# David-Wobrock/image-processing-graph-laplacian

Measured on AMD Instinct MI355X. Metric: filtered Mpixels/sec @ 4K img, 0.5% samples; PSNR vs PETSc ref, higher is better.
Workload: dtype f32 (f32 storage and accumulation; MFMA operands split into f16 hi+lo pairs = 22 significant bits)

## Files before the change

image-processing-graph-laplacian_amd/csrc/ctx.hip:

```cpp
#include "glf_internal.hpp"

#include <cmath>
#include <cstdlib>

extern "C" {

const char *glf_strerror(int status)
{
    switch (status) {
    case GLF_OK: return "ok";
    case GLF_ERR_INVALID: return "invalid argument";
    case GLF_ERR_NOMEM: return "out of memory";
    case GLF_ERR_HIP: return "HIP runtime error";
    case GLF_ERR_NODEVICE: return "no usable gfx950 device";
    case GLF_ERR_COMM: return "collective callback failed";
    case GLF_ERR_NOCONV: return "eigensolver did not converge";
    case GLF_ERR_IO: return "image I/O error";
    case GLF_ERR_UNSUPPORTED: return "unsupported";
    default: return "unknown status";
    }
}

int glf_ctx_create(glf_ctx **out, int device, void *hip_stream)
{
// ... 125 lines not shown
{
    if (!ctx) return GLF_OK;
    (void)hipSetDevice(ctx->device);
    (void)hipStreamSynchronize(ctx->stream);
    for (auto &e : ctx->ev)
        if (e) (void)hipEventDestroy(e);
    for (auto &row : ctx->mv_ev)
        for (auto &e : row)
            if (e) (void)hipEventDestroy(e);
    for (auto &row : ctx->cp_ev)
        for (auto &e : row)
            if (e) (void)hipEventDestroy(e);
    glf::native_comm_release(ctx);
    if (ctx->mv_scratch) (void)hipFree(ctx->mv_scratch);
    if (ctx->x0_block) (void)hipFree(ctx->x0_block);
    glf::band_cache_free(ctx);
    if (ctx->rank_ftab) (void)hipFree(ctx->rank_ftab);
    if (ctx->rank_ff) (void)hipFree(ctx->rank_ff);
    if (ctx->pinned) (void)hipHostFree(ctx->pinned);
    glf::pool_free_all(ctx, false);
    if (ctx->owns_stream && ctx->stream) (void)hipStreamDestroy(ctx->stream);
    delete ctx;
    return GLF_OK;
}

int glf_ctx_synchronize(glf_ctx *ctx)
{
    if (!ctx) return GLF_ERR_INVALID;
    GLF_HIP(ctx, hipStreamSynchronize(ctx->stream));
    return GLF_OK;
// ... 306 lines not shown
```

image-processing-graph-laplacian_amd/csrc/eigen.hip:

```cpp
#include "glf_internal.hpp"

#include <algorithm>
#include <cmath>
#include <cstdlib>
#include <cstring>

namespace glf {

typedef float f32x16 __attribute__((ext_vector_type(16)));


template <int MB>
__global__ __launch_bounds__(256) void k_block_matvec(const float *__restrict__ A, int64_t lda, unsigned p,
                                                       unsigned p32, const float *__restrict__ X,
                                                       float *__restrict__ Y)
{
    constexpr int LD = MB * 32;
    __shared__ __attribute__((aligned(16))) float xs[2][32 * LD];
    const int lane = threadIdx.x & 63, wave = threadIdx.x >> 6;
    const int half = lane >> 5, l31 = lane & 31;
    const unsigned row = blockIdx.x * 128 + wave * 32 + l31;
    const unsigned rowc = row < p ? row : p - 1;
    const float *arow = A + (size_t)rowc * lda + 16 * half;

// ... 336 lines not shown
    GLF_LAUNCH_CHECK(ctx);
    return GLF_OK;
}

int start_block_cached(glf_ctx *ctx, unsigned p, unsigned m, unsigned ld, unsigned long long seed, const float **d_block)
{
    if (!ctx->x0_block || ctx->x0_p != p || ctx->x0_m != m || ctx->x0_ld != ld || ctx->x0_seed != seed) {
        const size_t n = (size_t)round_up(p, VEC_PAD) * ld;
        std::vector<double> x0((size_t)m * p);
        glf_random_vectors(x0.data(), p, m, seed);
        std::vector<float> h(n, 0.f);
        for (unsigned j = 0; j < m; ++j)
            for (unsigned i = 0; i < p; ++i) h[(size_t)i * ld + j] = (float)x0[(size_t)j * p + i];
        if (ctx->x0_block) (void)hipFree(ctx->x0_block);
        ctx->x0_block = nullptr;
        GLF_HIP(ctx, hipMalloc(reinterpret_cast<void **>(&ctx->x0_block), n * sizeof(float)));
        GLF_HIP(ctx, hipMemcpyAsync(ctx->x0_block, h.data(), n * sizeof(float), hipMemcpyHostToDevice, ctx->stream));
        GLF_HIP(ctx, hipStreamSynchronize(ctx->stream));
        ctx->x0_p = p;
        ctx->x0_m = m;
        ctx->x0_ld = ld;
        ctx->x0_seed = seed;
    }
    *d_block = ctx->x0_block;
    return GLF_OK;
}

int mv_collect(glf_ctx *ctx)
{
    if (ctx->mv_pending == 0) return GLF_OK;
// ... 12 lines not shown
    unsigned r0 = 0, r1 = 0;
    bool dist = false;
    unsigned n() const { return r1 - r0; }
};
static inline Rows rows_of(unsigned p, const MatShard *sh)
{
    Rows r;
    if (sh && sh->rows_per_rank) {
        r.r0 = sh->row0;
        r.r1 = sh->row1;
        r.dist = true;
    } else {
        r.r1 = p;
    }
    return r;
}
static int allreduce_d(glf_ctx *ctx, double *d, size_t n)
{
    if (!ctx->has_comm || ctx->comm.allreduce_sum_f64(ctx->comm.user, d, n) != 0)
        return set_error(ctx, GLF_ERR_COMM, "allreduce_sum_f64 callback failed");
    return GLF_OK;
}
static int allreduce_f(glf_ctx *ctx, float *d, size_t n)
{
    if (!ctx->has_comm || ctx->comm.allreduce_sum_f32(ctx->comm.user, d, n) != 0)
        return set_error(ctx, GLF_ERR_COMM, "allreduce_sum_f32 callback failed");
    return GLF_OK;
}
static int allgather_rows(glf_ctx *ctx, float *V, const MatShard *sh, unsigned ld)
{
// ... 337 lines not shown
    {
        shard = sh;
        rows = rows_of(p, sh);
        const size_t n = (size_t)vec_rows(p, sh, ctx->comm.size) * ld;
        GLF_TRY(R.alloc(ctx, n));
        GLF_TRY(P.alloc(ctx, n));
        GLF_TRY(AP.alloc(ctx, n));
        GLF_TRY(Xs.alloc(ctx, n));
        GLF_TRY(dinv.alloc(ctx, p));
        nblk = (int)ceil_div(rows.n(), RED_ROWS);
        GLF_TRY(partial.alloc(ctx, (size_t)std::max(1, nblk) * 2 * ld));
        GLF_TRY(pmax.alloc(ctx, (size_t)std::max(1, nblk) * ld));
        GLF_TRY(sums.alloc(ctx, (size_t)2 * ld));
        GLF_TRY(scal.alloc(ctx, (size_t)4 * ld));
        GLF_TRY(flags.alloc(ctx, ld + 1));
        for (float *q : {R.p, P.p, AP.p, Xs.p}) GLF_HIP(ctx, hipMemsetAsync(q, 0, n * sizeof(float), ctx->stream));
        s.rz = scal.p;
        s.bn2 = scal.p + ld;
        s.alpha = scal.p + 2 * ld;
        s.beta = scal.p + 3 * ld;
        s.active = flags.p;
        if (!ctx_pinned(ctx)) return set_error(ctx, GLF_ERR_NOMEM, "pinned host page");
        h_nactive = reinterpret_cast<int *>(ctx_pinned(ctx) + PINNED_NACTIVE);
        s.nactive = h_nactive;
        return GLF_OK;
    }
};

static int block_pcg_work(glf_ctx *ctx, CgWork &w, const float *A, int64_t lda, unsigned p, float *XB, unsigned m,
                          unsigned ld, double rtol, int max_it, int *iters, bool solution_to_XB = true)
{
    const int nblk = w.nblk;
    const Rows rows = w.rows;
    const unsigned nloc = rows.n();
    const size_t off = (size_t)rows.r0 * ld;
    hipStream_t st = ctx->stream;
    const dim3 red2(red2_grid(ld)), red2_threads(RED2_THREADS);
    const bool carry = w.carry_maxima && !rows.dist;
    const ColMaxima pmax{w.pmax.p, nblk};
    auto reduce2 = [&](int nv, const double **src, int *src_blk) -> int {
        *src = w.partial.p;
        *src_blk = nblk;
        if (!rows.dist) return GLF_OK;
        if (nv == 1) hipLaunchKernelGGL(k_sum_partials_nv<1>, red2, red2_threads, 0, st, w.partial.p, nblk, ld, w.sums.p);
        else hipLaunchKernelGGL(k_sum_partials_nv<2>, red2, red2_threads, 0, st, w.partial.p, nblk, ld, w.sums.p);
// ... 1 lines not shown
        GLF_TRY(allreduce_d(ctx, w.sums.p, (size_t)nv * ld));
        *src = w.sums.p;
        *src_blk = 1;
        return GLF_OK;
    };
    const double *src = nullptr;
    int src_blk = 0;
    if (nblk > 0)
        hipLaunchKernelGGL(k_cg_init, dim3(nblk), dim3(256), 0, st, XB + off, w.dinv.p + rows.r0, w.R.p + off, w.P.p + off, w.Xs.p + off,
                           nloc, ld, w.partial.p, w.pmax.p);
    GLF_TRY(reduce2(2, &src, &src_blk));
    hipLaunchKernelGGL(k_cg_init_scalars, red2, red2_threads, 0, st, src, src_blk, ld, m, w.s);
    hipLaunchKernelGGL(k_cg_count, dim3(1), dim3(256), 0, st, w.s, ld);
    GLF_LAUNCH_CHECK(ctx);
    int it = 0;
    GLF_HIP(ctx, hipStreamSynchronize(st));
    while (*(volatile int *)w.h_nactive > 0 && it < max_it) {
        ++it;
        if (rows.dist) GLF_TRY(allgather_rows(ctx, w.P.p, w.shard, ld));
        unsigned wn = ld;
        if (w.shard && w.shard->grid && ld >= 64 && !ctx->tune.no_narrow) {
            const int na = *w.h_nactive;
            const unsigned cand = na <= 32 ? 32u : (unsigned)round_up(na, 64);
            if (cand < ld) wn = cand;
        }
        if (wn < ld) {
            if (!w.Pc.p) {
                const size_t n = (size_t)vec_rows(p, w.shard, ctx->comm.size) * ld;
                GLF_TRY(w.Pc.alloc(ctx, n));
                GLF_TRY(w.APc.alloc(ctx, n));
                GLF_TRY(w.pcmax.alloc(ctx, (size_t)ceil_div(p, RED_ROWS) * ld));
                GLF_HIP(ctx, hipMemsetAsync(w.Pc.p, 0, n * sizeof(float), st));
            }
            const ColMaxima pcmax{w.pcmax.p, (int)ceil_div(p, RED_ROWS)};
            hipLaunchKernelGGL(k_cg_pack, dim3((unsigned)pcmax.nblk), dim3(256), 0, st, w.P.p, w.s.active, p, ld, wn, w.Pc.p, w.pcmax.p);
            GLF_TRY(block_matvec(ctx, A, lda, p, w.Pc.p, w.APc.p, wn, w.shard, carry ? &pcmax : nullptr));
            if (nblk > 0)
// ... 3 lines not shown
        } else {
            GLF_TRY(block_matvec(ctx, A, lda, p, w.P.p, w.AP.p, ld, w.shard, carry ? &pmax : nullptr));
        }
        if (nblk > 0) hipLaunchKernelGGL(k_cg_dot, dim3(nblk), dim3(256), 0, st, w.P.p + off, w.AP.p + off, nloc, ld, w.partial.p);
        GLF_TRY(reduce2(1, &src, &src_blk));
        hipLaunchKernelGGL(k_cg_alpha, red2, red2_threads, 0, st, src, src_blk, ld, w.s);
        if (nblk > 0)
            hipLaunchKernelGGL(k_cg_update, dim3(nblk), dim3(256), 0, st, w.Xs.p + off, w.R.p + off, w.P.p + off, w.AP.p + off,
                               w.dinv.p + rows.r0, nloc, ld, w.s, w.partial.p);
        GLF_TRY(reduce2(2, &src, &src_blk));
        hipLaunchKernelGGL(k_cg_beta, red2, red2_threads, 0, st, src, src_blk, ld, rtol * rtol, w.s);
        hipLaunchKernelGGL(k_cg_pupdate, dim3((unsigned)std::max(1, nblk)), dim3(256), 0, st, w.P.p + off, w.R.p + off, w.dinv.p + rows.r0, nloc, ld,
                           w.s, carry ? w.pmax.p : nullptr);
        GLF_LAUNCH_CHECK(ctx);
        GLF_HIP(ctx, hipStreamSynchronize(st));
        if (ctx->tune.verbose) fprintf(stderr, "[glf] block PCG step %d: %d of %u columns active\n", it, *w.h_nactive, m);
    }
    if (nloc > 0 && solution_to_XB)
        GLF_HIP(ctx, hipMemcpyAsync(XB + off, w.Xs.p + off, sizeof(float) * (size_t)nloc * ld, hipMemcpyDeviceToDevice, st));
    if (iters) *iters = it;
    return (*w.h_nactive > 0) ? set_error(ctx, GLF_ERR_NOCONV, "block PCG: %d columns unconverged after %d iterations",
                                          *w.h_nactive, it)
                              : GLF_OK;
}

static int cg_setup(glf_ctx *ctx, CgWork &cg, const float *A, int64_t lda, unsigned p, unsigned ld, const MatShard *shard, const float *d_dinv)
{
    GLF_TRY(cg.init(ctx, p, ld, shard));
    cg.carry_maxima = true;
    if (d_dinv)
// ... 191 lines not shown
            b[u] = rowb[cb + u];
        }
#pragma unroll
        for (int u = 0; u < E; ++u)
#pragma unroll
            for (int v = 0; v < E; ++v) acc[u][v] = fma((double)a[u], (double)b[v], acc[u][v]);
    }
    double *out = Gpart + (size_t)blockIdx.x * ld * ld;
#pragma unroll
    for (int u = 0; u < E; ++u)
#pragma unroll
        for (int v = 0; v < E; ++v) out[(size_t)(ca + u) * ld + cb + v] = acc[u][v];
}

typedef double f64x4 __attribute__((ext_vector_type(4)));
template <int TILE>
__global__ __launch_bounds__(64) void k_gsf_gram_mfma(const float *__restrict__ X, unsigned n, unsigned ld,
                                                       double *__restrict__ Gpart, const float *__restrict__ Y = nullptr)
{
    constexpr int S = TILE / 16;
    const int mb = ld / TILE;
    const int ta = blockIdx.y / mb, tb = blockIdx.y % mb;
    if (!Y && tb < ta) return;
    const float *Yp = Y ? Y : X;
    const int lane = threadIdx.x, l15 = lane & 15, lq = lane >> 4;
    f64x4 acc[S][S];
#pragma unroll
    for (int u = 0; u < S; ++u)
#pragma unroll
        for (int v = 0; v < S; ++v)
#pragma unroll
            for (int r = 0; r < 4; ++r) acc[u][v][r] = 0.0;
    const unsigned r0 = blockIdx.x * GSF_ROWS, r1 = min(r0 + GSF_ROWS, n);
    const float *xa = X + ta * TILE + l15, *yb = Yp + tb * TILE + l15;
    const bool sym = !Y && ta == tb;
    for (unsigned ib = r0; ib < r1; ib += 32) {
        float a[8][S], b[8][S];
#pragma unroll
        for (int q = 0; q < 8; ++q) {
            const unsigned i = min(ib + 4 * q + lq, r1 - 1);
#pragma unroll
            for (int u = 0; u < S; ++u) {
                a[q][u] = xa[(size_t)i * ld + 16 * u];
                b[q][u] = yb[(size_t)i * ld + 16 * u];
            }
        }
#pragma unroll
        for (int q = 0; q < 8; ++q) {
            const bool ok = ib + 4 * q + lq < r1;
            double da[S], db[S];
#pragma unroll
            for (int u = 0; u < S; ++u) {
                da[u] = ok ? (double)a[q][u] : 0.0;
                db[u] = ok ? (double)b[q][u] : 0.0;
            }
#pragma unroll
            for (int u = 0; u < S; ++u)
#pragma unroll
                for (int v = 0; v < S; ++v)
                    if (!sym || v >= u) acc[u][v] = __builtin_amdgcn_mfma_f64_16x16x4f64(da[u], db[v], acc[u][v], 0, 0, 0);
        }
    }
    double *out = Gpart + (size_t)blockIdx.x * ld * ld;
#pragma unroll
    for (int u = 0; u < S; ++u)
#pragma unroll
        for (int v = 0; v < S; ++v) {
            if (sym && v < u) continue;
#pragma unroll
            for (int r = 0; r < 4; ++r) {
                const size_t ga = (size_t)(ta * TILE + 16 * u + lq + 4 * r), gb = (size_t)(tb * TILE + 16 * v + l15);
                out[ga * ld + gb] = acc[u][v][r];
                if (sym && v > u) out[gb * ld + ga] = acc[u][v][r];
            }
        }
}

__global__ __launch_bounds__(256) void k_gsf_sum(const double *__restrict__ Gpart, int nchunks, unsigned ld, int tile,
                                                  double *__restrict__ G, int full = 0)
{
    __shared__ double sh[256];
    const unsigned e = blockIdx.x * 64 + (threadIdx.x & 63);
    const int part = threadIdx.x >> 6;
    const unsigned a = e / ld, b = e % ld;
    const bool live = e < ld * ld && (full || b / tile >= a / tile);
    double s = 0.0;
    if (live) {
        int c = part;
        for (; c + 28 < nchunks; c += 32) {
            double x[8];
// ... 173 lines not shown
            const double tv = ts[j * ld + col];
#pragma unroll
            for (int q = 0; q < 8; ++q) acc[q] = fma((double)xs[(rl + q * nrl) * ld + j0 + j], tv, acc[q]);
        }
    }
    (void)rpt;
    if (col < m)
#pragma unroll
        for (int q = 0; q < 8; ++q) {
            const unsigned i = r0 + rl + q * nrl;
            if (i < n) Out[(size_t)i * ld + col] = (float)acc[q];
        }
}

template <int LD>
__global__ __launch_bounds__(256) void k_gsf_apply_mfma(const float *X, const float *__restrict__ S, float *Out, unsigned n, unsigned m,
                                                         const double *__restrict__ Tn, const int *__restrict__ flag, int tiles)
{
    if (*flag) return;
    constexpr int NTL = LD / 16, TS = LD + 4;
    __shared__ double ts[LD * TS];
    for (unsigned e = threadIdx.x; e < LD * LD; e += 256) ts[(e / LD) * TS + e % LD] = Tn[e];
    __syncthreads();
    const int lane = threadIdx.x & 63, wave = threadIdx.x >> 6, l15 = lane & 15, lq = lane >> 4;
#pragma unroll 1
    for (int tile = 0; tile < tiles; ++tile) {
        const unsigned row0 = (blockIdx.x * 4 * tiles + wave * tiles + tile) * 16;
        if (row0 >= n) break;
        const unsigned ra = min(row0 + l15, n - 1);
        float4 xa[NTL];
#pragma unroll
        for (int jb = 0; jb < NTL; ++jb) xa[jb] = *reinterpret_cast<const float4 *>(X + (size_t)ra * LD + 16 * jb + 4 * lq);
        if (S)
#pragma unroll
            for (int jb = 0; jb < NTL; ++jb) {
                const float4 s4 = *reinterpret_cast<const float4 *>(S + (size_t)ra * LD + 16 * jb + 4 * lq);
                xa[jb] = make_float4(xa[jb].x - s4.x, xa[jb].y - s4.y, xa[jb].z - s4.z, xa[jb].w - s4.w);
            }
        f64x4 acc[NTL];
#pragma unroll
        for (int t = 0; t < NTL; ++t)
#pragma unroll
            for (int r = 0; r < 4; ++r) acc[t][r] = 0.0;
#pragma unroll
        for (int jb = 0; jb < NTL; ++jb) {
            const double a4[4] = {(double)xa[jb].x, (double)xa[jb].y, (double)xa[jb].z, (double)xa[jb].w};
#pragma unroll
            for (int sk = 0; sk < 4; ++sk)
#pragma unroll
                for (int t = jb; t < NTL; ++t)
                    acc[t] = __builtin_amdgcn_mfma_f64_16x16x4f64(a4[sk], ts[(16 * jb + 4 * lq + sk) * TS + 16 * t + l15], acc[t], 0, 0, 0);
        }
#pragma unroll
        for (int t = 0; t < NTL; ++t)
#pragma unroll
            for (int r = 0; r < 4; ++r) {
                const unsigned i = row0 + lq + 4 * r;
                if (i < n && 16 * t + l15 < (int)m) Out[(size_t)i * LD + 16 * t + l15] = (float)acc[t][r];
            }
    }
}

__global__ __launch_bounds__(256) void k_gsf_sub(float *__restrict__ Y, const float *__restrict__ X, unsigned n, unsigned ld, unsigned ma,
                                                  const double *__restrict__ Cm)
{
    __shared__ float xs[GSF_APPLY_TILE];
    __shared__ double ts[4096];
    const unsigned rows = GSF_APPLY_TILE / ld, jb = min(4096u / ld, ld);
    const unsigned r0 = blockIdx.x * rows;
    const unsigned col = threadIdx.x % ld, rl = threadIdx.x / ld, nrl = 256 / ld;
    for (unsigned e = threadIdx.x; e < rows * ld; e += 256) {
        const unsigned i = r0 + e / ld;
        xs[e] = i < n ? X[(size_t)i * ld + e % ld] : 0.f;
    }
// ... 7 lines not shown
        const unsigned jn = min(jb, ma - j0);
        for (unsigned j = 0; j < jn; ++j) {
            const double tv = ts[j * ld + col];
#pragma unroll
            for (int q = 0; q < 8; ++q) acc[q] = fma((double)xs[(rl + q * nrl) * ld + j0 + j], tv, acc[q]);
        }
    }
#pragma unroll
    for (int q = 0; q < 8; ++q) {
        const unsigned i = r0 + rl + q * nrl;
        if (i < n) Y[(size_t)i * ld + col] = (float)((double)Y[(size_t)i * ld + col] - acc[q]);
    }
}

static void launch_gsf_apply(hipStream_t st, const float *X, const float *S, float *out, unsigned n, unsigned ld, unsigned m, const double *Tn,
                             const int *flag)
{
    const int tiles = (int)std::max<int64_t>(1, std::min<int64_t>(4, ceil_div(n, 16 * 4 * 256)));
    const unsigned rows_wg = 16 * 4 * (unsigned)tiles;
    if (ld == 64)
        hipLaunchKernelGGL(k_gsf_apply_mfma<64>, dim3((unsigned)ceil_div(n, rows_wg)), dim3(256), 0, st, X, S, out, n, m, Tn, flag, tiles);
    else if (ld == 32)
        hipLaunchKernelGGL(k_gsf_apply_mfma<32>, dim3((unsigned)ceil_div(n, rows_wg)), dim3(256), 0, st, X, S, out, n, m, Tn, flag, tiles);
    else
        hipLaunchKernelGGL(k_gsf_apply, dim3((unsigned)ceil_div(n, GSF_APPLY_TILE / ld)), dim3(256), 0, st, X, S, out, n, ld, m, Tn, flag);
}

struct GsFusedWork {
    DevBuf<double> Gpart, G, S, Tn;
    DevBuf<int> flag;
    int *h_flag = nullptr;
    int nchunks = 0;
    unsigned n = 0, ld = 0;
    int init(glf_ctx *ctx, unsigned n_, unsigned ld_)
    {
        if (n == n_ && ld == ld_) return GLF_OK;
        n = n_;
        ld = ld_;
        nchunks = (int)ceil_div(n, GSF_ROWS);
        GLF_TRY(Gpart.alloc(ctx, (size_t)std::max(1, nchunks) * ld * ld));
// ... 33 lines not shown
    const float *R;
    float *AX;
};

static int orthonormalise_fused_dev(glf_ctx *ctx, GsFusedWork &f, float *X, Rows rows, unsigned m, unsigned ld,
                                    double *d_norms, int *fell_back, const GsDerive *der = nullptr)
{
    hipStream_t st = ctx->stream;
    const unsigned n = rows.n();
    float *Xout = X + (size_t)rows.r0 * ld;
    const float *Xl = der ? der->Y + (size_t)rows.r0 * ld : Xout;
    GLF_TRY(f.init(ctx, n, ld));
    const int tile = ld >= 64 ? 64 : 32, mb = (int)ld / tile;
    if (f.nchunks > 0) {
        if (tile == 64)
            hipLaunchKernelGGL((k_gsf_gram_mfma<64>), dim3(f.nchunks, mb * mb), dim3(64), 0, st, Xl, n, ld, f.Gpart.p);
        else
            hipLaunchKernelGGL((k_gsf_gram_mfma<32>), dim3(f.nchunks, mb * mb), dim3(64), 0, st, Xl, n, ld, f.Gpart.p);
    }
    hipLaunchKernelGGL(k_gsf_sum, dim3((ld * ld + 63) / 64), dim3(256), 0, st, f.Gpart.p, f.nchunks, ld, tile, f.G.p);
    GLF_LAUNCH_CHECK(ctx);
    if (rows.dist) GLF_TRY(allreduce_d(ctx, f.G.p, (size_t)ld * ld));
    if (ld <= 64)
        hipLaunchKernelGGL(k_gsf_recur_lds, dim3(1), dim3(256), 0, st, ld, m, f.G.p, f.Tn.p, d_norms, f.flag.p, f.h_flag);
    else
        hipLaunchKernelGGL(k_gsf_recur_global, dim3(1), dim3(256), 0, st, ld, m, f.G.p, f.S.p, f.Tn.p, d_norms, f.flag.p, f.h_flag);
    if (n > 0 && der)
        launch_gsf_apply(st, Xout, der->R + (size_t)rows.r0 * ld, der->AX + (size_t)rows.r0 * ld, n, ld, m, f.Tn.p, f.flag.p);
    if (n > 0)
        launch_gsf_apply(st, Xl, nullptr, Xout, n, ld, m, f.Tn.p, f.flag.p);
    GLF_LAUNCH_CHECK(ctx);
    GLF_HIP(ctx, hipStreamSynchronize(st));
    *fell_back = *(volatile int *)f.h_flag;
    return GLF_OK;
}

static int orthonormalise_seq_dev(glf_ctx *ctx, GsWork &w, float *X, unsigned n, unsigned m, unsigned ld)
{
    hipStream_t st = ctx->stream;
    for (unsigned k = 0; k < m; ++k) {
        if (k > 0) {
            hipLaunchKernelGGL(k_gs_dots, dim3(w.nblk), dim3(256), 0, st, X, n, ld, k, w.partial.p);
            hipLaunchKernelGGL(k_gs_fin, dim3(k), dim3(256), 0, st, w.partial.p, w.normpart.p, w.nblk, ld, k, m, w.q.p, w.coef.p);
        }
        hipLaunchKernelGGL(k_gs_apply, dim3(w.nblk), dim3(256), 0, st, X, n, ld, k, w.nblk, w.coef.p, w.normpart.p);
    }
    hipLaunchKernelGGL(k_gs_fin, dim3(m), dim3(256), 0, st, w.partial.p, w.normpart.p, w.nblk, ld, m, m, w.q.p, w.coef.p);
    hipLaunchKernelGGL(k_gs_norms, dim3(1), dim3(256), 0, st, w.q.p, m, w.norms.p);
    hipLaunchKernelGGL(k_scale_all, dim3((unsigned)ceil_div((int64_t)n * ld, 256)), dim3(256), 0, st, X, n, ld, m, w.norms.p);
    GLF_LAUNCH_CHECK(ctx);
// ... 211 lines not shown

struct ResWork {
    DevBuf<float> AX, Gpart, G;
    DevBuf<double> partial, sums;
    double *h_sums = nullptr;
    int nchunks = 0;
    Rows rows;
    const MatShard *shard = nullptr;
    int init(glf_ctx *ctx, unsigned p, unsigned ld, const MatShard *sh = nullptr)
    {
        shard = sh;
        rows = rows_of(p, sh);
        const size_t vr = vec_rows(p, sh, ctx->comm.size);
        nchunks = (int)ceil_div(rows.n(), GRAM_ROWS);
        GLF_TRY(AX.alloc(ctx, vr * ld));
        GLF_HIP(ctx, hipMemsetAsync(AX.p, 0, sizeof(float) * vr * ld, ctx->stream));
        GLF_TRY(Gpart.alloc(ctx, (size_t)std::max(1, nchunks) * ld * ld));
        GLF_TRY(G.alloc(ctx, (size_t)ld * ld));
        GLF_TRY(partial.alloc(ctx, (size_t)std::max<int64_t>(1, ceil_div(rows.n(), RED_ROWS)) * ld));
        GLF_TRY(sums.alloc(ctx, ld));
        if (!ctx_pinned(ctx) || ld > 256) return set_error(ctx, GLF_ERR_NOMEM, "pinned host page");
        h_sums = reinterpret_cast<double *>(ctx_pinned(ctx) + PINNED_SUMS);
        return GLF_OK;
    }
};

static int residual_dev(glf_ctx *ctx, ResWork &w, const float *A, int64_t lda, unsigned p, float *X, unsigned m,
                        unsigned ld, double *h_out, bool ax_ready = false)
{
    const Rows rows = w.rows;
    const unsigned nloc = rows.n();
// ... 42 lines not shown
                            const double *h_X0, int opti_gs, double epsilon, double inner_rtol, int max_outer,
                            float *d_eigvecs, double *h_eigvals, glf_eig_stats *stats, const MatShard *shard,
                            const float *d_dinv, const float *d_X0_block)
{
    if (m == 0 || m > p || !valid_ld(ld) || m > ld)
        return set_error(ctx, GLF_ERR_INVALID, "inverse_power_iteration: m=%u ld=%u p=%u (m <= 256 supported)", m, ld, p);
    if (opti_gs < 1) opti_gs = 1;
    const unsigned p32 = (unsigned)round_up(p, VEC_PAD);
    const size_t n = (size_t)vec_rows(p, shard, ctx->comm.size) * ld;
    const size_t n_out = (size_t)p32 * ld;
    hipStream_t st = ctx->stream;

    DevBuf<float> X, Xb;
    GLF_TRY(X.alloc(ctx, n));
    GLF_TRY(Xb.alloc(ctx, n));
    if (d_X0_block) {
        GLF_HIP(ctx, hipMemsetAsync(X.p, 0, sizeof(float) * n, st));
        GLF_HIP(ctx, hipMemcpyAsync(X.p, d_X0_block, sizeof(float) * n_out, hipMemcpyDeviceToDevice, st));
    } else {
        std::vector<double> own;
        if (!h_X0) {
            own.resize((size_t)m * p);
            glf_random_vectors(own.data(), p, m, 1);
            h_X0 = own.data();
        }
        std::vector<float> h(n, 0.f);
        for (unsigned j = 0; j < m; ++j)
            for (unsigned i = 0; i < p; ++i) h[(size_t)i * ld + j] = (float)h_X0[(size_t)j * p + i];
        GLF_HIP(ctx, hipMemcpyAsync(X.p, h.data(), sizeof(float) * n, hipMemcpyHostToDevice, st));
        GLF_HIP(ctx, hipStreamSynchronize(st));
    }
    GsWork gs;
    GLF_TRY(gs.init(ctx, p, ld));
    CgWork cg;
    GLF_TRY(cg_setup(ctx, cg, A, lda, p, ld, shard, d_dinv));
    ResWork rs;
    GLF_TRY(rs.init(ctx, p, ld, shard));
    const Rows rows = rows_of(p, shard);
    const unsigned nloc = rows.n();
    const size_t off = (size_t)rows.r0 * ld, nloc_ld = (size_t)nloc * ld;
    GLF_TRY(mv_collect(ctx));
    const int mv_count0 = ctx->mv_count, narrow0 = ctx->narrow_sweeps;
    const double mv_ms0 = ctx->mv_ms, mv_bytes0 = ctx->mv_bytes;
    bool replicated = false;
    GLF_TRY(orthonormalise_dev(ctx, gs, X.p, p, m, ld, rows, shard, &replicated));
    GLF_HIP(ctx, hipMemcpyAsync(Xb.p, X.p, sizeof(float) * n, hipMemcpyDeviceToDevice, st));
    double r_norm = 0.0;
    GLF_TRY(residual_dev(ctx, rs, A, lda, p, X.p, m, ld, &r_norm));
    const bool verbose = ctx->tune.verbose;
    if (verbose) fprintf(stderr, "[glf rank %d] initial residual %.9g\n", ctx->comm.rank, r_norm);
    int it = 0, inner_total = 0, rc = GLF_OK;
    const bool derive_ax = !ctx->tune.residual_sweep;
    const bool swap_blocks = derive_ax && !ctx->tune.gs_seq && opti_gs == 1 && !rows.dist;
    while (r_norm > epsilon) {
        if (it >= max_outer) {
            rc = set_error(ctx, GLF_ERR_NOCONV, "inverse iteration: residual %g > %g after %d outer iterations", r_norm,
                           epsilon, it);
            break;
        }
        ++it;
        int inner = 0;
        bool ax_ready = derive_ax;
        if (swap_blocks) {
            GLF_TRY(block_pcg_work(ctx, cg, A, lda, p, X.p, m, ld, inner_rtol, 10 * (int)p + 100, &inner, false));
            inner_total += inner;
            const GsDerive der{cg.Xs.p, cg.R.p, rs.AX.p};
            int fell_back = 0;
            GLF_TRY(orthonormalise_fused_dev(ctx, gs.fused, X.p, rows, m, ld, gs.norms.p, &fell_back, &der));
            gs.last_fused = !fell_back;
            if (fell_back) {
                if (verbose) fprintf(stderr, "[glf] Gram-Schmidt: ill-conditioned block, column-by-column sweep\n");
                GLF_HIP(ctx, hipMemcpyAsync(X.p, cg.Xs.p, sizeof(float) * nloc_ld, hipMemcpyDeviceToDevice, st));
                GLF_TRY(orthonormalise_seq_dev(ctx, gs, X.p, p, m, ld));
                ax_ready = false;
            }
            std::swap(cg.Xs.p, Xb.p);
        } else {
            if (derive_ax && nloc) GLF_HIP(ctx, hipMemcpyAsync(rs.AX.p + off, X.p + off, sizeof(float) * nloc_ld, hipMemcpyDeviceToDevice, st));
            GLF_TRY(block_pcg_work(ctx, cg, A, lda, p, X.p, m, ld, inner_rtol, 10 * (int)p + 100, &inner));
            inner_total += inner;
            if (nloc) GLF_HIP(ctx, hipMemcpyAsync(Xb.p + off, X.p + off, sizeof(float) * nloc_ld, hipMemcpyDeviceToDevice, st));
            if (derive_ax && nloc)
                hipLaunchKernelGGL(k_sub_inplace, dim3((unsigned)ceil_div((int64_t)nloc_ld, 256)), dim3(256), 0, st, rs.AX.p + off, cg.R.p + off, nloc_ld);
            if (it % opti_gs == 0) {
                GLF_TRY(orthonormalise_dev(ctx, gs, X.p, p, m, ld, rows, shard, &replicated));
                if (ax_ready && gs.last_fused) {
                    if (nloc) launch_gsf_apply(st, rs.AX.p + off, nullptr, rs.AX.p + off, nloc, ld, m, gs.fused.Tn.p, gs.fused.flag.p);
                } else {
                    ax_ready = false;
                }
            }
        }
        GLF_LAUNCH_CHECK(ctx);
        GLF_TRY(residual_dev(ctx, rs, A, lda, p, X.p, m, ld, &r_norm, ax_ready));
        if (verbose)
            fprintf(stderr, "[glf rank %d] outer iteration %d: %d block-CG steps, residual %.9g\n", ctx->comm.rank, it, inner, r_norm);
    }
    if (opti_gs != 1 && (it % opti_gs) != 0)
        GLF_TRY(orthonormalise_dev(ctx, gs, X.p, p, m, ld, rows, shard, &replicated));

    if (h_eigvals) {
        std::vector<double> nr(m);
        GLF_HIP(ctx, hipMemcpyAsync(nr.data(), gs.norms.p, sizeof(double) * m, hipMemcpyDeviceToHost, st));
        GLF_HIP(ctx, hipStreamSynchronize(st));
        for (unsigned j = 0; j < m; ++j) h_eigvals[j] = 1.0 / nr[j];
    }
    if (d_eigvecs) {
        GLF_TRY(normalise_dev(ctx, Xb.p, p, m, ld, gs.partial.p, gs.norms.p, rows, cg.sums.p));
        if (rows.dist) GLF_TRY(allgather_rows(ctx, Xb.p, shard, ld));
        GLF_HIP(ctx, hipMemcpyAsync(d_eigvecs, Xb.p, sizeof(float) * n_out, hipMemcpyDeviceToDevice, st));
    }
    GLF_HIP(ctx, hipStreamSynchronize(st));
// ... 215 lines not shown
```

image-processing-graph-laplacian_amd/csrc/glf_internal.hpp:

```cpp
#pragma once

#include <hip/hip_runtime.h>

#include <cmath>
#include <cstdarg>
#include <cstdint>
#include <cstdio>
#include <cstring>
#include <limits>
#include <type_traits>
#include <utility>
#include <vector>

#include "../../include/glf.h"
#include "band_plan.hpp"

struct glf_pool_block {
    void *p;
    size_t bytes;
    bool in_use;
    unsigned last_call = 0;
};

struct glf_tuning {
// ... 35 lines not shown
    hipEvent_t ev[8] = {};
    void *mv_scratch = nullptr;
    size_t mv_scratch_bytes = 0;
    static constexpr int MV_RING = 64;
    hipEvent_t mv_ev[2][MV_RING] = {};
    static constexpr int CP_RING = 16;
    hipEvent_t cp_ev[2][CP_RING] = {};
    int mv_pending = 0;
    unsigned call_no = 0;
    int mv_count = 0;
    int narrow_sweeps = 0;
    double mv_ms = 0.0, mv_bytes = 0.0;
    float *x0_block = nullptr;
    unsigned x0_p = 0, x0_m = 0, x0_ld = 0;
    unsigned long long x0_seed = 0;
    int contraction = GLF_CONTRACT_F16_SPLIT;
    struct { int skipping = 0, lut = 0; } nys_note;
    struct { int path = 0, shape = 0, skipping = 0, chunks = 0, mgroups = 0; double entries = 0.0; } deg_note;
    struct { unsigned kernels = 0, ld = 0, panels = 0, proj_blocks = 0, apply_blocks = 0, strided = 0; } flt_note;
    void *pinned = nullptr;
    void *band_cache[2] = {nullptr, nullptr};
    bool rank_valid = false;
    float rank_s_val = 0.f;
    int rank_R = 0;
    void *rank_ftab = nullptr;
    void *rank_ff = nullptr;
    bool pool_debug = false;
    int pool_violations = 0;
    glf_tuning tune;
};
// ... 662 lines not shown
```

Measured before the change: 2648.

## Cut eigensolver syncs, cache orthonormal start block, widen Gram kernel, fuse apply passes

Several eigensolver changes land together. The orthonormalised random start block and its norms are cached across calls, since they depend only on the seed and shape. The first block-PCG step skips its host sync, the fused Gram-Schmidt no longer waits on its fallback flag before the residual is launched, and buffer memsets now clear only the padding rows. The Gram kernel spreads its MFMA tile pairs over four waves, and the apply kernel writes both orthonormalised outputs in one launch. Together these aim to remove host round trips and redundant passes, at the cost of more control-flow complexity and an extra persistent cache that must be invalidated correctly.

```diff
diff --git a/image-processing-graph-laplacian_amd/csrc/ctx.hip b/image-processing-graph-laplacian_amd/csrc/ctx.hip
--- a/image-processing-graph-laplacian_amd/csrc/ctx.hip
+++ b/image-processing-graph-laplacian_amd/csrc/ctx.hip
@@ -163,6 +163,8 @@
     glf::native_comm_release(ctx);
     if (ctx->mv_scratch) (void)hipFree(ctx->mv_scratch);
     if (ctx->x0_block) (void)hipFree(ctx->x0_block);
+    if (ctx->x0_orth) (void)hipFree(ctx->x0_orth);
+    if (ctx->x0_orth_norms) (void)hipFree(ctx->x0_orth_norms);
     glf::band_cache_free(ctx);
     if (ctx->rank_ftab) (void)hipFree(ctx->rank_ftab);
     if (ctx->rank_ff) (void)hipFree(ctx->rank_ff);
diff --git a/image-processing-graph-laplacian_amd/csrc/eigen.hip b/image-processing-graph-laplacian_amd/csrc/eigen.hip
--- a/image-processing-graph-laplacian_amd/csrc/eigen.hip
+++ b/image-processing-graph-laplacian_amd/csrc/eigen.hip
@@ -374,6 +374,7 @@
             for (unsigned i = 0; i < p; ++i) h[(size_t)i * ld + j] = (float)x0[(size_t)j * p + i];
         if (ctx->x0_block) (void)hipFree(ctx->x0_block);
         ctx->x0_block = nullptr;
+        ctx->x0_orth_form = 0;
         GLF_HIP(ctx, hipMalloc(reinterpret_cast<void **>(&ctx->x0_block), n * sizeof(float)));
         GLF_HIP(ctx, hipMemcpyAsync(ctx->x0_block, h.data(), n * sizeof(float), hipMemcpyHostToDevice, ctx->stream));
         GLF_HIP(ctx, hipStreamSynchronize(ctx->stream));
@@ -416,6 +417,11 @@
         r.r1 = p;
     }
     return r;
+}
+static int zero_pad_rows(glf_ctx *ctx, float *q, size_t from, size_t rows, unsigned ld)
+{
+    if (from < rows) GLF_HIP(ctx, hipMemsetAsync(q + from * ld, 0, (rows - from) * ld * sizeof(float), ctx->stream));
+    return GLF_OK;
 }
 static int allreduce_d(glf_ctx *ctx, double *d, size_t n)
 {
@@ -783,7 +789,8 @@
         GLF_TRY(sums.alloc(ctx, (size_t)2 * ld));
         GLF_TRY(scal.alloc(ctx, (size_t)4 * ld));
         GLF_TRY(flags.alloc(ctx, ld + 1));
-        for (float *q : {R.p, P.p, AP.p, Xs.p}) GLF_HIP(ctx, hipMemsetAsync(q, 0, n * sizeof(float), ctx->stream));
+        const bool may_narrow = sh && sh->grid && ld >= 64 && !ctx->tune.no_narrow;
+        for (float *q : {R.p, P.p, AP.p, Xs.p}) GLF_TRY(zero_pad_rows(ctx, q, (rows.dist || (q == AP.p && may_narrow)) ? 0 : p, n / ld, ld));
         s.rz = scal.p;
         s.bn2 = scal.p + ld;
         s.alpha = scal.p + 2 * ld;
@@ -797,7 +804,7 @@
 };
 
 static int block_pcg_work(glf_ctx *ctx, CgWork &w, const float *A, int64_t lda, unsigned p, float *XB, unsigned m,
-                          unsigned ld, double rtol, int max_it, int *iters, bool solution_to_XB = true)
+                          unsigned ld, double rtol, int max_it, int *iters, bool solution_to_XB = true, bool rhs_active = false)
 {
     const int nblk = w.nblk;
     const Rows rows = w.rows;
@@ -829,13 +836,14 @@
     hipLaunchKernelGGL(k_cg_count, dim3(1), dim3(256), 0, st, w.s, ld);
     GLF_LAUNCH_CHECK(ctx);
     int it = 0;
-    GLF_HIP(ctx, hipStreamSynchronize(st));
-    while (*(volatile int *)w.h_nactive > 0 && it < max_it) {
+    bool unsynced = rhs_active && !rows.dist && !ctx->tune.verbose && max_it > 0;
+    if (!unsynced) GLF_HIP(ctx, hipStreamSynchronize(st));
+    while ((unsynced || *(volatile int *)w.h_nactive > 0) && it < max_it) {
         ++it;
         if (rows.dist) GLF_TRY(allgather_rows(ctx, w.P.p, w.shard, ld));
         unsigned wn = ld;
         if (w.shard && w.shard->grid && ld >= 64 && !ctx->tune.no_narrow) {
-            const int na = *w.h_nactive;
+            const int na = unsynced ? (int)m : *w.h_nactive;
             const unsigned cand = na <= 32 ? 32u : (unsigned)round_up(na, 64);
             if (cand < ld) wn = cand;
         }
@@ -869,6 +877,7 @@
                            w.s, carry ? w.pmax.p : nullptr);
         GLF_LAUNCH_CHECK(ctx);
         GLF_HIP(ctx, hipStreamSynchronize(st));
+        unsynced = false;
         if (ctx->tune.verbose) fprintf(stderr, "[glf] block PCG step %d: %d of %u columns active\n", it, *w.h_nactive, m);
     }
     if (nloc > 0 && solution_to_XB)
@@ -1090,66 +1099,91 @@
 }
 
 typedef double f64x4 __attribute__((ext_vector_type(4)));
+constexpr int GSF_GRAM_WAVES = 4;
+template <int S, bool SYM>
+__host__ __device__ constexpr int gsf_pair_index(int u, int v)
+{
+    return SYM ? u * S - u * (u - 1) / 2 + (v - u) : u * S + v;
+}
+template <int TILE, bool SYM, int W>
+__device__ __forceinline__ void gsf_gram_wave(const float *__restrict__ xa, const float *__restrict__ yb, unsigned ld, unsigned r0,
+                                              unsigned r1, int lq, int l15, int ca, int cb, double *__restrict__ out)
+{
+    constexpr int S = TILE / 16;
+    auto mine = [](int u, int v) { return (!SYM || v >= u) && gsf_pair_index<S, SYM>(u, v) % GSF_GRAM_WAVES == W; };
+    f64x4 acc[S][S];
+#pragma unroll
+    for (int u = 0; u < S; ++u)
+#pragma unroll
+        for (int v = 0; v < S; ++v)
+#pragma unroll
+            for (int r = 0; r < 4; ++r) acc[u][v][r] = 0.0;
+    for (unsigned ib = r0; ib < r1; ib += 32) {
+        float a[8][S], b[8][S];
+#pragma unroll
+        for (int q = 0; q < 8; ++q) {
+            const unsigned i = min(ib + 4 * q + lq, r1 - 1);
+#pragma unroll
+            for (int u = 0; u < S; ++u) {
+                a[q][u] = xa[(size_t)i * ld + 16 * u];
+                b[q][u] = SYM ? a[q][u] : yb[(size_t)i * ld + 16 * u];
+            }
+        }
+#pragma unroll
+        for (int q = 0; q < 8; ++q) {
+            const bool ok = ib + 4 * q + lq < r1;
+            double da[S], db[S];
+#pragma unroll
+            for (int u = 0; u < S; ++u) {
+                da[u] = ok ? (double)a[q][u] : 0.0;
+                db[u] = ok ? (double)b[q][u] : 0.0;
+            }
+#pragma unroll
+            for (int u = 0; u < S; ++u)
+#pragma unroll
+                for (int v = 0; v < S; ++v)
+                    if (mine(u, v)) acc[u][v] = __builtin_amdgcn_mfma_f64_16x16x4f64(da[u], db[v], acc[u][v], 0, 0, 0);
+        }
+    }
+#pragma unroll
+    for (int u = 0; u < S; ++u)
+#pragma unroll
+        for (int v = 0; v < S; ++v) {
+            if (!mine(u, v)) continue;
+#pragma unroll
+            for (int r = 0; r < 4; ++r) {
+                const size_t ga = (size_t)(ca + 16 * u + lq + 4 * r), gb = (size_t)(cb + 16 * v + l15);
+                out[ga * ld + gb] = acc[u][v][r];
+                if (SYM && v > u) out[gb * ld + ga] = acc[u][v][r];
+            }
+        }
+}
 template <int TILE>
-__global__ __launch_bounds__(64) void k_gsf_gram_mfma(const float *__restrict__ X, unsigned n, unsigned ld,
-                                                       double *__restrict__ Gpart, const float *__restrict__ Y = nullptr)
-{
-    constexpr int S = TILE / 16;
+__global__ __launch_bounds__(64 * GSF_GRAM_WAVES) void k_gsf_gram_mfma(const float *__restrict__ X, unsigned n, unsigned ld,
+                                                                        double *__restrict__ Gpart, const float *__restrict__ Y = nullptr)
+{
     const int mb = ld / TILE;
     const int ta = blockIdx.y / mb, tb = blockIdx.y % mb;
     if (!Y && tb < ta) return;
     const float *Yp = Y ? Y : X;
-    const int lane = threadIdx.x, l15 = lane & 15, lq = lane >> 4;
-    f64x4 acc[S][S];
-#pragma unroll
-    for (int u = 0; u < S; ++u)
-#pragma unroll
-        for (int v = 0; v < S; ++v)
-#pragma unroll
-            for (int r = 0; r < 4; ++r) acc[u][v][r] = 0.0;
+    const int lane = threadIdx.x & 63, wave = threadIdx.x >> 6, l15 = lane & 15, lq = lane >> 4;
     const unsigned r0 = blockIdx.x * GSF_ROWS, r1 = min(r0 + GSF_ROWS, n);
     const float *xa = X + ta * TILE + l15, *yb = Yp + tb * TILE + l15;
+    double *out = Gpart + (size_t)blockIdx.x * ld * ld;
     const bool sym = !Y && ta == tb;
-    for (unsigned ib = r0; ib < r1; ib += 32) {
-        float a[8][S], b[8][S];
-#pragma unroll
-        for (int q = 0; q < 8; ++q) {
-            const unsigned i = min(ib + 4 * q + lq, r1 - 1);
-#pragma unroll
-            for (int u = 0; u < S; ++u) {
-                a[q][u] = xa[(size_t)i * ld + 16 * u];
-                b[q][u] = yb[(size_t)i * ld + 16 * u];
-            }
-        }
-#pragma unroll
-        for (int q = 0; q < 8; ++q) {
-            const bool ok = ib + 4 * q + lq < r1;
-            double da[S], db[S];
-#pragma unroll
-            for (int u = 0; u < S; ++u) {
-                da[u] = ok ? (double)a[q][u] : 0.0;
-                db[u] = ok ? (double)b[q][u] : 0.0;
-            }
-#pragma unroll
-            for (int u = 0; u < S; ++u)
-#pragma unroll
-                for (int v = 0; v < S; ++v)
-                    if (!sym || v >= u) acc[u][v] = __builtin_amdgcn_mfma_f64_16x16x4f64(da[u], db[v], acc[u][v], 0, 0, 0);
-        }
-    }
-    double *out = Gpart + (size_t)blockIdx.x * ld * ld;
-#pragma unroll
-    for (int u = 0; u < S; ++u)
-#pragma unroll
-        for (int v = 0; v < S; ++v) {
-            if (sym && v < u) continue;
-#pragma unroll
-            for (int r = 0; r < 4; ++r) {
-                const size_t ga = (size_t)(ta * TILE + 16 * u + lq + 4 * r), gb = (size_t)(tb * TILE + 16 * v + l15);
-                out[ga * ld + gb] = acc[u][v][r];
-                if (sym && v > u) out[gb * ld + ga] = acc[u][v][r];
-            }
-        }
+#define GLF_GSF_GRAM_WAVE(W)                                                                                          \
+    case W:                                                                                                           \
+        if (sym) gsf_gram_wave<TILE, true, W>(xa, yb, ld, r0, r1, lq, l15, ta * TILE, tb * TILE, out);                \
+        else gsf_gram_wave<TILE, false, W>(xa, yb, ld, r0, r1, lq, l15, ta * TILE, tb * TILE, out);                   \
+        break;
+    static_assert(GSF_GRAM_WAVES == 4, "one case per wave below");
+    switch (wave) {
+        GLF_GSF_GRAM_WAVE(0)
+        GLF_GSF_GRAM_WAVE(1)
+        GLF_GSF_GRAM_WAVE(2)
+        GLF_GSF_GRAM_WAVE(3)
+    }
+#undef GLF_GSF_GRAM_WAVE
 }
 
 __global__ __launch_bounds__(256) void k_gsf_sum(const double *__restrict__ Gpart, int nchunks, unsigned ld, int tile,
@@ -1353,8 +1387,36 @@
 }
 
 template <int LD>
-__global__ __launch_bounds__(256) void k_gsf_apply_mfma(const float *X, const float *__restrict__ S, float *Out, unsigned n, unsigned m,
-                                                         const double *__restrict__ Tn, const int *__restrict__ flag, int tiles)
+__device__ __forceinline__ void gsf_apply_tile(const float4 (&xa)[LD / 16], const double *ts, float *Out, unsigned row0, unsigned n,
+                                               unsigned m, int lq, int l15)
+{
+    constexpr int NTL = LD / 16, TS = LD + 4;
+    f64x4 acc[NTL];
+#pragma unroll
+    for (int t = 0; t < NTL; ++t)
+#pragma unroll
+        for (int r = 0; r < 4; ++r) acc[t][r] = 0.0;
+#pragma unroll
+    for (int jb = 0; jb < NTL; ++jb) {
+        const double a4[4] = {(double)xa[jb].x, (double)xa[jb].y, (double)xa[jb].z, (double)xa[jb].w};
+#pragma unroll
+        for (int sk = 0; sk < 4; ++sk)
+#pragma unroll
+            for (int t = jb; t < NTL; ++t)
+                acc[t] = __builtin_amdgcn_mfma_f64_16x16x4f64(a4[sk], ts[(16 * jb + 4 * lq + sk) * TS + 16 * t + l15], acc[t], 0, 0, 0);
+    }
+#pragma unroll
+    for (int t = 0; t < NTL; ++t)
+#pragma unroll
+        for (int r = 0; r < 4; ++r) {
+            const unsigned i = row0 + lq + 4 * r;
+            if (i < n && 16 * t + l15 < (int)m) Out[(size_t)i * LD + 16 * t + l15] = (float)acc[t][r];
+        }
+}
+template <int LD>
+__global__ __launch_bounds__(256) void k_gsf_apply_mfma(const float *X, const float *__restrict__ S, float *Out, const float *X2, float *Out2,
+                                                         unsigned n, unsigned m, const double *__restrict__ Tn,
+                                                         const int *__restrict__ flag, int tiles)
 {
     if (*flag) return;
     constexpr int NTL = LD / 16, TS = LD + 4;
@@ -1367,36 +1429,20 @@
         const unsigned row0 = (blockIdx.x * 4 * tiles + wave * tiles + tile) * 16;
         if (row0 >= n) break;
         const unsigned ra = min(row0 + l15, n - 1);
-        float4 xa[NTL];
+        float4 xa[NTL], xb[NTL];
 #pragma unroll
         for (int jb = 0; jb < NTL; ++jb) xa[jb] = *reinterpret_cast<const float4 *>(X + (size_t)ra * LD + 16 * jb + 4 * lq);
+        if (X2)
+#pragma unroll
+            for (int jb = 0; jb < NTL; ++jb) xb[jb] = *reinterpret_cast<const float4 *>(X2 + (size_t)ra * LD + 16 * jb + 4 * lq);
         if (S)
 #pragma unroll
             for (int jb = 0; jb < NTL; ++jb) {
                 const float4 s4 = *reinterpret_cast<const float4 *>(S + (size_t)ra * LD + 16 * jb + 4 * lq);
                 xa[jb] = make_float4(xa[jb].x - s4.x, xa[jb].y - s4.y, xa[jb].z - s4.z, xa[jb].w - s4.w);
             }
-        f64x4 acc[NTL];
-#pragma unroll
-        for (int t = 0; t < NTL; ++t)
-#pragma unroll
-            for (int r = 0; r < 4; ++r) acc[t][r] = 0.0;
-#pragma unroll
-        for (int jb = 0; jb < NTL; ++jb) {
-            const double a4[4] = {(double)xa[jb].x, (double)xa[jb].y, (double)xa[jb].z, (double)xa[jb].w};
-#pragma unroll
-            for (int sk = 0; sk < 4; ++sk)
-#pragma unroll
-                for (int t = jb; t < NTL; ++t)
-                    acc[t] = __builtin_amdgcn_mfma_f64_16x16x4f64(a4[sk], ts[(16 * jb + 4 * lq + sk) * TS + 16 * t + l15], acc[t], 0, 0, 0);
-        }
-#pragma unroll
-        for (int t = 0; t < NTL; ++t)
-#pragma unroll
-            for (int r = 0; r < 4; ++r) {
-                const unsigned i = row0 + lq + 4 * r;
-                if (i < n && 16 * t + l15 < (int)m) Out[(size_t)i * LD + 16 * t + l15] = (float)acc[t][r];
-            }
+        gsf_apply_tile<LD>(xa, ts, Out, row0, n, m, lq, l15);
+        if (X2) gsf_apply_tile<LD>(xb, ts, Out2, row0, n, m, lq, l15);
     }
 }
 
@@ -1434,16 +1480,18 @@
 }
 
 static void launch_gsf_apply(hipStream_t st, const float *X, const float *S, float *out, unsigned n, unsigned ld, unsigned m, const double *Tn,
-                             const int *flag)
+                             const int *flag, const float *X2 = nullptr, float *out2 = nullptr)
 {
     const int tiles = (int)std::max<int64_t>(1, std::min<int64_t>(4, ceil_div(n, 16 * 4 * 256)));
     const unsigned rows_wg = 16 * 4 * (unsigned)tiles;
     if (ld == 64)
-        hipLaunchKernelGGL(k_gsf_apply_mfma<64>, dim3((unsigned)ceil_div(n, rows_wg)), dim3(256), 0, st, X, S, out, n, m, Tn, flag, tiles);
+        hipLaunchKernelGGL(k_gsf_apply_mfma<64>, dim3((unsigned)ceil_div(n, rows_wg)), dim3(256), 0, st, X, S, out, X2, out2, n, m, Tn, flag, tiles);
     else if (ld == 32)
-        hipLaunchKernelGGL(k_gsf_apply_mfma<32>, dim3((unsigned)ceil_div(n, rows_wg)), dim3(256), 0, st, X, S, out, n, m, Tn, flag, tiles);
-    else
+        hipLaunchKernelGGL(k_gsf_apply_mfma<32>, dim3((unsigned)ceil_div(n, rows_wg)), dim3(256), 0, st, X, S, out, X2, out2, n, m, Tn, flag, tiles);
+    else {
         hipLaunchKernelGGL(k_gsf_apply, dim3((unsigned)ceil_div(n, GSF_APPLY_TILE / ld)), dim3(256), 0, st, X, S, out, n, ld, m, Tn, flag);
+        if (X2) hipLaunchKernelGGL(k_gsf_apply, dim3((unsigned)ceil_div(n, GSF_APPLY_TILE / ld)), dim3(256), 0, st, X2, nullptr, out2, n, ld, m, Tn, flag);
+    }
 }
 
 struct GsFusedWork {
@@ -1507,9 +1555,9 @@
     const int tile = ld >= 64 ? 64 : 32, mb = (int)ld / tile;
     if (f.nchunks > 0) {
         if (tile == 64)
-            hipLaunchKernelGGL((k_gsf_gram_mfma<64>), dim3(f.nchunks, mb * mb), dim3(64), 0, st, Xl, n, ld, f.Gpart.p);
+            hipLaunchKernelGGL((k_gsf_gram_mfma<64>), dim3(f.nchunks, mb * mb), dim3(64 * GSF_GRAM_WAVES), 0, st, Xl, n, ld, f.Gpart.p);
         else
-            hipLaunchKernelGGL((k_gsf_gram_mfma<32>), dim3(f.nchunks, mb * mb), dim3(64), 0, st, Xl, n, ld, f.Gpart.p);
+            hipLaunchKernelGGL((k_gsf_gram_mfma<32>), dim3(f.nchunks, mb * mb), dim3(64 * GSF_GRAM_WAVES), 0, st, Xl, n, ld, f.Gpart.p);
     }
     hipLaunchKernelGGL(k_gsf_sum, dim3((ld * ld + 63) / 64), dim3(256), 0, st, f.Gpart.p, f.nchunks, ld, tile, f.G.p);
     GLF_LAUNCH_CHECK(ctx);
@@ -1519,14 +1567,16 @@
     else
         hipLaunchKernelGGL(k_gsf_recur_global, dim3(1), dim3(256), 0, st, ld, m, f.G.p, f.S.p, f.Tn.p, d_norms, f.flag.p, f.h_flag);
     if (n > 0 && der)
-        launch_gsf_apply(st, Xout, der->R + (size_t)rows.r0 * ld, der->AX + (size_t)rows.r0 * ld, n, ld, m, f.Tn.p, f.flag.p);
-    if (n > 0)
+        launch_gsf_apply(st, Xout, der->R + (size_t)rows.r0 * ld, der->AX + (size_t)rows.r0 * ld, n, ld, m, f.Tn.p, f.flag.p, Xl, Xout);
+    else if (n > 0)
         launch_gsf_apply(st, Xl, nullptr, Xout, n, ld, m, f.Tn.p, f.flag.p);
     GLF_LAUNCH_CHECK(ctx);
+    if (!fell_back) return GLF_OK;
     GLF_HIP(ctx, hipStreamSynchronize(st));
     *fell_back = *(volatile int *)f.h_flag;
     return GLF_OK;
 }
+static inline int gsf_fell_back(const GsFusedWork &f) { return *(volatile int *)f.h_flag; }
 
 static int orthonormalise_seq_dev(glf_ctx *ctx, GsWork &w, float *X, unsigned n, unsigned m, unsigned ld)
 {
@@ -1768,7 +1818,7 @@
         const size_t vr = vec_rows(p, sh, ctx->comm.size);
         nchunks = (int)ceil_div(rows.n(), GRAM_ROWS);
         GLF_TRY(AX.alloc(ctx, vr * ld));
-        GLF_HIP(ctx, hipMemsetAsync(AX.p, 0, sizeof(float) * vr * ld, ctx->stream));
+        GLF_TRY(zero_pad_rows(ctx, AX.p, rows.dist ? 0 : p, vr, ld));
         GLF_TRY(Gpart.alloc(ctx, (size_t)std::max(1, nchunks) * ld * ld));
         GLF_TRY(G.alloc(ctx, (size_t)ld * ld));
         GLF_TRY(partial.alloc(ctx, (size_t)std::max<int64_t>(1, ceil_div(rows.n(), RED_ROWS)) * ld));
@@ -1841,9 +1891,13 @@
     DevBuf<float> X, Xb;
     GLF_TRY(X.alloc(ctx, n));
     GLF_TRY(Xb.alloc(ctx, n));
+    const Rows rows = rows_of(p, shard);
+    const bool start_cached = d_X0_block && d_X0_block == ctx->x0_block && ctx->x0_p == p && ctx->x0_m == m && ctx->x0_ld == ld && !rows.dist;
+    const int start_form = 1 + (ctx->tune.gs_seq ? 1 : 0);
+    const bool start_hit = start_cached && ctx->x0_orth_form == start_form;
     if (d_X0_block) {
-        GLF_HIP(ctx, hipMemsetAsync(X.p, 0, sizeof(float) * n, st));
-        GLF_HIP(ctx, hipMemcpyAsync(X.p, d_X0_block, sizeof(float) * n_out, hipMemcpyDeviceToDevice, st));
+        GLF_TRY(zero_pad_rows(ctx, X.p, p32, n / ld, ld));
+        GLF_HIP(ctx, hipMemcpyAsync(X.p, start_hit ? ctx->x0_orth : d_X0_block, sizeof(float) * n_out, hipMemcpyDeviceToDevice, st));
     } else {
         std::vector<double> own;
         if (!h_X0) {
@@ -1863,15 +1917,36 @@
     GLF_TRY(cg_setup(ctx, cg, A, lda, p, ld, shard, d_dinv));
     ResWork rs;
     GLF_TRY(rs.init(ctx, p, ld, shard));
-    const Rows rows = rows_of(p, shard);
     const unsigned nloc = rows.n();
     const size_t off = (size_t)rows.r0 * ld, nloc_ld = (size_t)nloc * ld;
     GLF_TRY(mv_collect(ctx));
     const int mv_count0 = ctx->mv_count, narrow0 = ctx->narrow_sweeps;
     const double mv_ms0 = ctx->mv_ms, mv_bytes0 = ctx->mv_bytes;
     bool replicated = false;
-    GLF_TRY(orthonormalise_dev(ctx, gs, X.p, p, m, ld, rows, shard, &replicated));
-    GLF_HIP(ctx, hipMemcpyAsync(Xb.p, X.p, sizeof(float) * n, hipMemcpyDeviceToDevice, st));
+    if (start_hit) {
+        GLF_HIP(ctx, hipMemcpyAsync(gs.norms.p, ctx->x0_orth_norms, sizeof(double) * ld, hipMemcpyDeviceToDevice, st));
+        gs.last_fused = ctx->x0_orth_fused;
+    } else {
+        GLF_TRY(orthonormalise_dev(ctx, gs, X.p, p, m, ld, rows, shard, &replicated));
+        if (start_cached) {
+            if (!ctx->x0_orth_form) {
+                if (ctx->x0_orth) (void)hipFree(ctx->x0_orth);
+                if (ctx->x0_orth_norms) (void)hipFree(ctx->x0_orth_norms);
+                ctx->x0_orth = nullptr;
+                ctx->x0_orth_norms = nullptr;
+                GLF_HIP(ctx, hipMalloc(reinterpret_cast<void **>(&ctx->x0_orth), n_out * sizeof(float)));
+                GLF_HIP(ctx, hipMalloc(reinterpret_cast<void **>(&ctx->x0_orth_norms), ld * sizeof(double)));
+            }
+            ctx->x0_orth_form = 0;
+            GLF_HIP(ctx, hipMemcpyAsync(ctx->x0_orth, X.p, sizeof(float) * n_out, hipMemcpyDeviceToDevice, st));
+            GLF_HIP(ctx, hipMemcpyAsync(ctx->x0_orth_norms, gs.norms.p, sizeof(double) * ld, hipMemcpyDeviceToDevice, st));
+            ctx->x0_orth_fused = gs.last_fused;
+            ctx->x0_orth_form = start_form;
+        }
+    }
+    const bool xb_late = !rows.dist;
+    if (xb_late) GLF_TRY(zero_pad_rows(ctx, Xb.p, p, n / ld, ld));
+    else GLF_HIP(ctx, hipMemcpyAsync(Xb.p, X.p, sizeof(float) * n, hipMemcpyDeviceToDevice, st));
     double r_norm = 0.0;
     GLF_TRY(residual_dev(ctx, rs, A, lda, p, X.p, m, ld, &r_norm));
     const bool verbose = ctx->tune.verbose;
@@ -1889,19 +1964,26 @@
         int inner = 0;
         bool ax_ready = derive_ax;
         if (swap_blocks) {
-            GLF_TRY(block_pcg_work(ctx, cg, A, lda, p, X.p, m, ld, inner_rtol, 10 * (int)p + 100, &inner, false));
+            GLF_TRY(block_pcg_work(ctx, cg, A, lda, p, X.p, m, ld, inner_rtol, 10 * (int)p + 100, &inner, false, true));
             inner_total += inner;
             const GsDerive der{cg.Xs.p, cg.R.p, rs.AX.p};
-            int fell_back = 0;
-            GLF_TRY(orthonormalise_fused_dev(ctx, gs.fused, X.p, rows, m, ld, gs.norms.p, &fell_back, &der));
-            gs.last_fused = !fell_back;
-            if (fell_back) {
+            GLF_TRY(orthonormalise_fused_dev(ctx, gs.fused, X.p, rows, m, ld, gs.norms.p, nullptr, &der));
+            std::swap(cg.Xs.p, Xb.p);
+            rc = residual_dev(ctx, rs, A, lda, p, X.p, m, ld, &r_norm, true);
+            if (rc != GLF_OK) {
+                (void)hipStreamSynchronize(st);
+                return rc;
+            }
+            gs.last_fused = !gsf_fell_back(gs.fused);
+            if (!gs.last_fused) {
                 if (verbose) fprintf(stderr, "[glf] Gram-Schmidt: ill-conditioned block, column-by-column sweep\n");
-                GLF_HIP(ctx, hipMemcpyAsync(X.p, cg.Xs.p, sizeof(float) * nloc_ld, hipMemcpyDeviceToDevice, st));
+                GLF_HIP(ctx, hipMemcpyAsync(X.p, Xb.p, sizeof(float) * nloc_ld, hipMemcpyDeviceToDevice, st));
                 GLF_TRY(orthonormalise_seq_dev(ctx, gs, X.p, p, m, ld));
-                ax_ready = false;
+                GLF_TRY(residual_dev(ctx, rs, A, lda, p, X.p, m, ld, &r_norm, false));
             }
-            std::swap(cg.Xs.p, Xb.p);
+            if (verbose)
+                fprintf(stderr, "[glf rank %d] outer iteration %d: %d block-CG steps, residual %.9g\n", ctx->comm.rank, it, inner, r_norm);
+            continue;
         } else {
             if (derive_ax && nloc) GLF_HIP(ctx, hipMemcpyAsync(rs.AX.p + off, X.p + off, sizeof(float) * nloc_ld, hipMemcpyDeviceToDevice, st));
             GLF_TRY(block_pcg_work(ctx, cg, A, lda, p, X.p, m, ld, inner_rtol, 10 * (int)p + 100, &inner));
@@ -1923,6 +2005,7 @@
         if (verbose)
             fprintf(stderr, "[glf rank %d] outer iteration %d: %d block-CG steps, residual %.9g\n", ctx->comm.rank, it, inner, r_norm);
     }
+    if (xb_late && it == 0) GLF_HIP(ctx, hipMemcpyAsync(Xb.p, X.p, sizeof(float) * n, hipMemcpyDeviceToDevice, st));
     if (opti_gs != 1 && (it % opti_gs) != 0)
         GLF_TRY(orthonormalise_dev(ctx, gs, X.p, p, m, ld, rows, shard, &replicated));
 
diff --git a/image-processing-graph-laplacian_amd/csrc/glf_internal.hpp b/image-processing-graph-laplacian_amd/csrc/glf_internal.hpp
--- a/image-processing-graph-laplacian_amd/csrc/glf_internal.hpp
+++ b/image-processing-graph-laplacian_amd/csrc/glf_internal.hpp
@@ -73,6 +73,10 @@
     float *x0_block = nullptr;
     unsigned x0_p = 0, x0_m = 0, x0_ld = 0;
     unsigned long long x0_seed = 0;
+    float *x0_orth = nullptr;
+    double *x0_orth_norms = nullptr;
+    int x0_orth_form = 0;
+    bool x0_orth_fused = false;
     int contraction = GLF_CONTRACT_F16_SPLIT;
     struct { int skipping = 0, lut = 0; } nys_note;
     struct { int path = 0, shape = 0, skipping = 0, chunks = 0, mgroups = 0; double entries = 0.0; } deg_note;
```

New measurement: 2825, median of 6. 1.07x the previous value.
